# jackhwalters/DCS-Net

Measured on AMD Instinct MI355X. Metric: STFT frames/sec (train fwd+bwd+Adam), higher is better.
Workload: dtype f32

## Files before the change

### dcs-net_amd/csrc/lstm.hip

```cpp
#include "dcs_common.h"

namespace {

typedef float v2f __attribute__((ext_vector_type(2)));

__device__ __forceinline__ float fast_tanh(float x) {
    return 1.f - 2.f * __builtin_amdgcn_rcpf(__builtin_amdgcn_exp2f(x * 2.885390081777927f) + 1.f);
}

__device__ __forceinline__ void step_barrier() { asm volatile("s_waitcnt lgkmcnt(0)\n\ts_barrier" ::: "memory"); }

template <int CTRL>
__device__ __forceinline__ float quad_dpp(float v) { return dcs_dpp_term<CTRL, 0xf>(v); }
__device__ __forceinline__ float quad_bcast0(float v) { return quad_dpp<0x00>(v); }
__device__ __forceinline__ float quad_bcast1(float v) { return quad_dpp<0x55>(v); }
__device__ __forceinline__ float quad_bcast2(float v) { return quad_dpp<0xAA>(v); }
__device__ __forceinline__ float quad_bcast3(float v) { return quad_dpp<0xFF>(v); }
__device__ __forceinline__ float quad_sum(float v) {
    v += quad_dpp<0xB1>(v);
    v += quad_dpp<0x4E>(v);
    return v;
}

template <int H, bool SAVE>
// ... 152 lines not shown
}

extern "C" int dcs_lstm_layer_fwd_bias(const float* gx, const float* w_hh, const float* bias_a, const float* bias_b, float* out,
                                       float* gates_save, float* c_save, float* hprev_save, int n_sets, int seqs_per_set, int S,
                                       int Hdim, long stride_set, long stride_n, long stride_t, dcs_stream_t stream) {
    if (!gx || !w_hh || !out || n_sets <= 0 || seqs_per_set <= 0 || S <= 0 || (Hdim != 64 && Hdim != 128)) return DCS_ERR_BADARG;
    if ((gates_save == nullptr) != (c_save == nullptr)) return DCS_ERR_BADARG;
    if (bias_b && !bias_a) return DCS_ERR_BADARG;
    const int NS = n_sets * seqs_per_set;
    dim3 grid(NS * 2);
    if (Hdim == 128 && gates_save)
        DCS_LAUNCH((lstm_rec_fwd_kernel<128, true>), grid, dim3(512), 0, dcs_stream(stream), gx, w_hh, out, gates_save,
                           c_save, hprev_save, S, seqs_per_set, stride_set, stride_n, stride_t, bias_a, bias_b);
    else if (Hdim == 128)
        DCS_LAUNCH((lstm_rec_fwd_kernel<128, false>), grid, dim3(512), 0, dcs_stream(stream), gx, w_hh, out, gates_save,
                           c_save, hprev_save, S, seqs_per_set, stride_set, stride_n, stride_t, bias_a, bias_b);
    else if (gates_save)
        DCS_LAUNCH((lstm_rec_fwd_kernel<64, true>), grid, dim3(256), 0, dcs_stream(stream), gx, w_hh, out, gates_save,
                           c_save, hprev_save, S, seqs_per_set, stride_set, stride_n, stride_t, bias_a, bias_b);
    else
        DCS_LAUNCH((lstm_rec_fwd_kernel<64, false>), grid, dim3(256), 0, dcs_stream(stream), gx, w_hh, out, gates_save,
                           c_save, hprev_save, S, seqs_per_set, stride_set, stride_n, stride_t, bias_a, bias_b);
    DCS_CHECK_LAUNCH();
    return DCS_OK;
}

extern "C" int dcs_lstm_layer_fwd(const float* gx, const float* w_hh, float* out, float* gates_save, float* c_save,
                                  float* hprev_save, int n_sets, int seqs_per_set, int S, int Hdim, long stride_set, long stride_n,
                                  long stride_t, dcs_stream_t stream) {
    return dcs_lstm_layer_fwd_bias(gx, w_hh, nullptr, nullptr, out, gates_save, c_save, hprev_save, n_sets, seqs_per_set, S, Hdim,
                                   stride_set, stride_n, stride_t, stream);
}


namespace {
__global__ __launch_bounds__(256) void lstm_combine_fwd_kernel(const float* __restrict__ o, float2* __restrict__ out, long n) {
    const long i = (long)blockIdx.x * 256 + threadIdx.x;
    if (i >= n) return;
    const float rr = o[i], ir = o[n + i], ri = o[2 * n + i], ii = o[3 * n + i];
    out[i] = make_float2(rr - ii, ir + ri);
}
__global__ __launch_bounds__(256) void lstm_combine_bwd_kernel(const float2* __restrict__ g, float* __restrict__ g_o, long n) {
    DCS_PRIO_CRITICAL();
    const long i = (long)blockIdx.x * 256 + threadIdx.x;
    if (i >= n) return;
    const float2 v = g[i];
    g_o[i] = v.x; g_o[n + i] = v.y; g_o[2 * n + i] = v.y; g_o[3 * n + i] = -v.x;
}
__global__ __launch_bounds__(256) void lstm_param_grads_kernel(const float* __restrict__ part, const float* __restrict__ b_part,
                                                                float* __restrict__ g_whh, float* __restrict__ g_bih,
                                                                float* __restrict__ g_bhh, int CK, int seqs, int H, int w_blocks,
                                                                const float* __restrict__ part_ih, float* __restrict__ g_wih,
                                                                int CK_ih, long MN_ih, int ih_blocks, int ih_first) {
    if ((int)blockIdx.x >= ih_first) {
        const int bx = blockIdx.x - ih_first, s_ = bx / ih_blocks;
        const long i = (long)(bx % ih_blocks) * 256 + threadIdx.x;
        if (i >= MN_ih) return;
        const float* q = part_ih + (long)s_ * CK_ih * MN_ih + i;
        float a = 0.f;
#pragma unroll 8
        for (int c = 0; c < CK_ih; ++c) a += q[(long)c * MN_ih];
        g_wih[s_ * MN_ih + i] += a;
        return;
    }
    const int WH = 4 * H * H, nW = 4 * WH;
    if ((int)blockIdx.x < w_blocks) {
// ... 168 lines not shown
```

### dcs-net_amd/dcsnet/_lib.py

```python
import ctypes
import os

_HERE = os.path.dirname(os.path.abspath(__file__))
LIB_PATH = os.environ.get('DCS_LIB_PATH') or os.path.join(os.path.dirname(_HERE), 'lib', 'libdcsnet_hip.so')

ACT_NONE, ACT_RELU, ACT_LRELU, ACT_SIGMOID = 0, 1, 2, 3

_P = ctypes.c_void_p
_I = ctypes.c_int
_L = ctypes.c_long
_F = ctypes.c_float
_U64 = ctypes.c_ulonglong



class AttentionItem(ctypes.Structure):
    _fields_ = [(n, _P) for n in ('x', 'w1', 'w2', 'wsa', 'sa_bias', 'ca', 'pooled', 'hidden', 'sp', 'sa', 'y', 'g_out',
                                  'wsa_bwd', 'g_pre', 'g_sp', 'g_x', 'g_fc0_r', 'g_fc0_i', 'g_fc2_r', 'g_fc2_i')] + \
               [(n, _I) for n in ('H', 'W', 'C', 'Ch')] + [('g_pooled', _P)]


class SnapshotItem(ctypes.Structure):
    _fields_ = [('src', _P), ('words', _L), ('dst_word', _L), ('is_f32', _I), ('pad_', _I)]

# ... 22 lines not shown
    'dcs_cconv2d_bwd_weight_workspace_bytes': (_L, [_I] * 14),
    'dcs_cconv2d_bwd_weight': (_I, [_P] * 8 + [_L] + [_I] * 15 + [_P]),
    'dcs_cbn_workspace_bytes': (_L, [_L, _I]),
    'dcs_cbn_fwd': (_I, [_P] * 9 + [_L, _L, _I, _F, _F, _I, _I, _F, _U64, _P, _P]),
    'dcs_cbn_fwd_slabs': (_I, [_P] * 9 + [_I, _I, _P, _L, _I, _F, _F, _I, _F, _U64, _P, _P]),
    'dcs_ca_pool_chunks': (_I, [_L, _I]),
    'dcs_cbn_fwd_slabs_pool': (_I, [_P] * 9 + [_I, _I, _P, _P, _L, _I, _L, _I, _F, _F, _I, _P]),
    'dcs_channel_attention_fc_fwd': (_I, [_P] * 6 + [_I, _L, _I, _I, _P]),
    'dcs_cbn_bwd_workspace_bytes': (_L, [_L, _I]),
    'dcs_cbn_bwd': (_I, [_P] * 9 + [_L, _L, _I, _I, _I, _F, _U64, _P, _P]),
    'dcs_cbn_bwd_add': (_I, [_P] * 9 + [_L, _L, _I, _I, _I, _F, _U64, _P, _P, _F, _L, _P, _P]),
    'dcs_ca_workspace_bytes': (_L, [_I, _L, _I]),
    'dcs_channel_attention_fwd': (_I, [_P] * 7 + [_L, _I, _L, _I, _I, _P]),
    'dcs_spatial_pool_fwd': (_I, [_P, _P, _P, _I, _L, _I, _P]),
    'dcs_attention_apply_fwd': (_I, [_P, _P, _P, _P, _I, _L, _I, _F, _U64, _P, _P]),
    'dcs_rattention_workspace_bytes': (_L, [_I, _L, _I]),
    'dcs_rattention_fwd': (_I, [_P] * 8 + [_L] + [_I] * 6 + [_P]),
    'dcs_rattention_train_workspace_bytes': (_L, [_I, _L, _I, _I]),
    'dcs_rattention_pool_fwd': (_I, [_P] * 8 + [_L] + [_I] * 5 + [_P]),
    'dcs_rattention_apply_fwd': (_I, [_P] * 4 + [_I] * 4 + [_P]),
    'dcs_rattention_apply_bwd': (_I, [_P] * 8 + [_L] + [_I] * 4 + [_P]),
    'dcs_rattention_pool_bwd': (_I, [_P] * 11 + [_I] + [_P, _L] + [_I] * 5 + [_P]),
    'dcs_attention_bwd_sa': (_I, [_P] * 5 + [_I, _L, _I, _F, _U64, _P, _P]),
    'dcs_attention_bwd_workspace_bytes': (_L, [_I, _L, _I, _I]),
    'dcs_attention_bwd_x': (_I, [_P] * 16 + [_L, _I, _L, _I, _I, _F, _U64, _P, _P]),
    'dcs_attention_bwd_fc_weights': (_I, [_P, _L, _P, _P, _P, _P, _P, _P, _I, _L, _I, _I, _P]),
    'dcs_attention_fwd_batched_workspace_bytes': (_L, [_I, _P, _I]),
    'dcs_attention_fwd_batched': (_I, [_I, _P, _P, _L, _I, _P]),
    'dcs_attention_bwd_batched_workspace_bytes': (_L, [_I, _P, _I]),
    'dcs_attention_bwd_batched': (_I, [_I, _P, _P, _L, _I, _P]),
    'dcs_lstm_layer_fwd': (_I, [_P] * 6 + [_I, _I, _I, _I, _L, _L, _L, _P]),
    'dcs_lstm_layer_fwd_bias': (_I, [_P, _P, _P, _P, _P, _P, _P, _P, _I, _I, _I, _I, _L, _L, _L, _P]),
    'dcs_lstm_layer_bwd': (_I, [_P] * 6 + [_I] * 4 + [_P]),
    'dcs_dropout_fwd': (_I, [_P, _P, _L, _F, _U64, _P, _P]),
    'dcs_complex_act_fwd': (_I, [_P, _P, _L, _I, _P]),
    'dcs_complex_upsample_fwd': (_I, [_P, _P, _I, _I, _I, _I, _I, _I, _P]),
    'dcs_tapsum_fwd': (_I, [_P, _P, _P, _P] + [_I] * 10 + [_P]),
    'dcs_cconv_up2_single_fwd': (_I, [_P] * 6 + [_I] * 6 + [_P]),
    'dcs_cconv_up2_single_bwd_data': (_I, [_P] * 4 + [_I] * 6 + [_P]),
    'dcs_cconv_up2_single_bwd_weight_workspace_bytes': (_L, []),
    'dcs_cconv_up2_single_bwd_weight': (_I, [_P] * 7 + [_I, _P, _L] + [_I] * 5 + [_P]),
    'dcs_tapsum_bwd_workspace_bytes': (_L, []),
    'dcs_tapsum_bwd': (_I, [_P, _P, _P, _P, _P, _L] + [_I] * 10 + [_P]),
    'dcs_bound_crm_fwd': (_I, [_P, _P, _L, _F, _P]),
    'dcs_bound_mask_apply_fwd': (_I, [_P, _P, _P, _P, _P, _L, _F, _P]),
    'dcs_bound_mask_apply_bwd': (_I, [_P] * 6 + [_L, _F, _P]),
    'dcs_bound2_mask_apply_fwd': (_I, [_P] * 6 + [_L, _F, _F, _U64, _P, _P]),
    'dcs_bound2_mask_apply_bwd': (_I, [_P] * 7 + [_L, _F, _F, _U64, _P, _P]),
    'dcs_bound2_apply_polar_frames_fwd': (_I, [_P] * 4 + [_I] * 4 + [_F, _F, _U64, _P, _P]),
    'dcs_bound2_apply_polar_frames_bwd': (_I, [_P] * 5 + [_I] * 4 + [_F, _I, _F, _U64, _P, _P]),
    'dcs_complex_abs_f32': (_I, [_P, _P, _L, _P]),
    'dcs_rmask_apply_polar_frames_fwd': (_I, [_P] * 4 + [_I] * 4 + [_F, _I, _P]),
    'dcs_rmask_apply_polar_frames_bwd': (_I, [_P] * 5 + [_I] * 4 + [_F, _I, _I, _P]),
    'dcs_irfft512_frames': (_I, [_P, _P, _L, _P]),
    'dcs_rfft512_frames': (_I, [_P, _P, _L, _P]),
    'dcs_rfft512_ola_frames': (_I, [_P, _P, _P, _P, _I, _I, _I, _F, _P]),
    'dcs_irfft512_ola_frames': (_I, [_P, _P, _P, _P, _I, _I, _I, _F, _P]),
    'dcs_polar_frames_fwd': (_I, [_P, _P, _I, _I, _I, _I, _F, _P]),
    'dcs_polar_frames_bwd': (_I, [_P, _P, _P, _I, _I, _I, _I, _F, _I, _P]),
    'dcs_istft_envelope': (_I, [_P, _P, _I, _I, _I, _P]),
    'dcs_istft_ola_fwd': (_I, [_P, _P, _P, _P, _I, _I, _I, _I, _F, _P]),
    'dcs_istft_ola_bwd': (_I, [_P, _P, _P, _P, _I, _I, _I, _I, _F, _P]),
    'dcs_stft_frames_fwd': (_I, [_P, _P, _P, _P, _I, _I, _I, _I, _I, _P]),
    'dcs_stft_bins_fwd': (_I, [_P, _P, _I, _I, _I, _F, _P]),
    'dcs_sisnr_fwd': (_I, [_P, _P, _P, _P, _I, _I, _F, _P]),
    'dcs_sisnr_bwd': (_I, [_P, _P, _P, _P, _F, _P, _I, _I, _P]),
# ... 100 lines not shown
```

### dcs-net_amd/dcsnet/functional.py

```python
import os
import weakref

import torch

from . import _derived
from . import ops
from .ops import ACT_NONE, ACT_RELU, ACT_LRELU, ACT_SIGMOID, to_nhwc, from_nhwc
from ._lib import DcsHipError

_PACKED = _derived.Derived(capacity=512)


def bump_param_generation():
    _derived.bump_generation()
    ops.pack_plan_invalidate()


def note_state_update():
    _derived.bump_generation()


state_generation = _derived.generation


# ... 478 lines not shown


def _project_bwd(g_gx, w_ih, shared):
    G8, K = w_ih.shape[1], w_ih.shape[2]
    M = g_gx.shape[1]
    if not (ops.gemm_ok(M, K, G8, 2, True) and g_gx.is_contiguous() and w_ih.is_contiguous()):
        if shared:
            g_inp = torch.mm(g_gx[0], w_ih[0])
            return g_inp.addmm_(g_gx[1], w_ih[1])
        return torch.bmm(g_gx, w_ih)
    if shared:
        g_inp = torch.empty((M, K), dtype=torch.float32, device=g_gx.device)
        return ops.gemm_f32(g_gx, w_ih, g_inp, M, K, G8, G8, K, K, False, nseg=2, a_seg=M * G8, b_seg=G8 * K)
    g_inp = torch.empty((2, M, K), dtype=torch.float32, device=g_gx.device)
    return ops.gemm_f32(g_gx, w_ih, g_inp, M, K, G8, G8, K, K, False, nbatch=2, a_batch=M * G8, b_batch=G8 * K, c_batch=M * K)


class _ProjectFn(torch.autograd.Function):

    @staticmethod
    def forward(ctx, inp, w_ih):
        ctx.save_for_backward(inp, w_ih)
        return _project(inp, w_ih, shared=inp.dim() == 2, per_set=True)

    @staticmethod
    def backward(ctx, g):
        inp, w_ih = ctx.saved_tensors
        g = g.contiguous()
        g_inp = _project_bwd(g, w_ih, shared=inp.dim() == 2) if ctx.needs_input_grad[0] else None
        g_w = torch.matmul(g.transpose(1, 2), inp) if ctx.needs_input_grad[1] else None
        return g_inp, g_w


class _LstmLayerFn(torch.autograd.Function):

    @staticmethod
    def forward(ctx, inp, anchor, st, B2, S):
        w_ih, w_hh = st['weight_ih'][0], st['weight_hh'][0]
        need = inp.requires_grad or anchor.requires_grad
        ctx.planes = 0
        if inp.is_complex():
            zr = torch.view_as_real(inp)
            G8, K = w_ih.shape[1], w_ih.shape[2]
            ctx.planes = R0 = zr.shape[0] * zr.shape[1]
            gx = torch.empty((2 * R0, 2 * G8), dtype=torch.float32, device=inp.device)
            ops.gemm_f32(zr, w_ih, gx, 2 * R0, 2 * G8, K, K, K, 2 * G8, True, a_planes=R0)
            inp = zr
            G4 = G8 // 2
            strides = (G8, S * 2 * G8, 2 * G8)
        elif inp.dim() == 2:
            G8 = w_ih.shape[1]
            gx = _project(inp, w_ih, shared=True)
            G4 = G8 // 2
            strides = (G8, S * 2 * G8, 2 * G8)
        else:
            gx = _project(inp, w_ih, shared=False)
            G4 = gx.shape[-1] // 2
            strides = (B2 * S * 2 * G4, S * 2 * G4, 2 * G4)
        out, gates, c, hprev = ops.lstm_layer(gx, w_hh, 2, B2, S, strides, need, True,
                                              bias=(st['bias_ih'][0], st['bias_hh'][0]))
        ctx.st, ctx.dims = st, (B2, S)
        if need:
            ctx.save_for_backward(inp, hprev, gates, c)
        return out

    @staticmethod
    def backward(ctx, g_out):
        global sink_hits
        inp, hprev, gates, c = ctx.saved_tensors
        st, (B2, S) = ctx.st, ctx.dims
        w_ih, w_hh = st['weight_ih'][0], st['weight_hh'][0]
        H = w_hh.shape[-1]
        NT = B2 * S
# ... 67 lines not shown
    return st


_LSTM_OPERANDS = _derived.Derived()


def _lstm_layer_operands(sets, layer):
    names = [f'_l{layer}', f'_l{layer}_reverse']
    params = [getattr(m, k + n) for m in sets for n in names for k in ('weight_ih', 'weight_hh', 'bias_ih', 'bias_hh')]

    def make():
        w_ih = torch.stack([torch.cat([getattr(m, 'weight_ih' + n) for n in names]) for m in sets])
        bias = torch.stack([torch.cat([getattr(m, 'bias_ih' + n) + getattr(m, 'bias_hh' + n) for n in names])
                            for m in sets])
        w_hh = torch.stack([torch.stack([getattr(m, 'weight_hh' + n) for n in names]) for m in sets]).contiguous()
        return w_ih, bias, w_hh
    cacheable = not (torch.is_grad_enabled() and any(p.requires_grad for p in params))
    if not cacheable:
        return make()
    return _LSTM_OPERANDS.get(sets[0], layer, params, lambda: tuple(t.detach() for t in make()))


def complex_lstm(z, real_lstm, imag_lstm):
    if not (real_lstm.bidirectional and real_lstm.batch_first and real_lstm.hidden_size == 64):
        raise DcsHipError('complex_lstm: the HIP path implements the reference geometry '
                          '(bidirectional, batch_first, hidden 64: c_network.py:118-123)')
    B, S, I = z.shape
    sets = (real_lstm, imag_lstm)
    inp = None
    stacked = _stacked_lstm(real_lstm) if torch.is_grad_enabled() else None
    in_place = (stacked is not None and z.is_contiguous() and (B * S) % 64 == 0 and I % 64 == 0
                and ops.gemm_ok(2 * B * S, 16 * real_lstm.hidden_size, I, 1, True) and ops.gemm_ok(2 * B * S, I, 8 * real_lstm.hidden_size, 2, True)
                and stacked[0]['weight_ih'][0].is_contiguous() and stacked[0]['weight_ih'][1].is_contiguous())
    x2 = None if in_place else torch.view_as_real(z).permute(3, 0, 1, 2).reshape(2 * B * S, I)
    for layer in range(real_lstm.num_layers):
        if stacked is not None:
            out = _LstmLayerFn.apply((z if in_place else x2) if layer == 0 else inp, real_lstm.weight_ih_l0, stacked[layer], 2 * B, S)
            inp = out.view(2, 2 * B * S, -1)
            continue
        w_ih, bias, w_hh = _lstm_layer_operands(sets, layer)
        if not (torch.is_grad_enabled() and ((x2 if layer == 0 else inp).requires_grad or bias.requires_grad or w_ih.requires_grad)):
            if layer == 0:
                G8 = w_ih.shape[1]
                gx = _project(x2, w_ih.contiguous(), shared=True, train=False)
                strides = (G8, S * 2 * G8, 2 * G8)
            else:
                gx = _project(inp, w_ih.contiguous(), shared=False, train=False)
                strides = (2 * B * S * gx.shape[-1], S * gx.shape[-1], gx.shape[-1])
            out = ops.lstm_layer(gx, w_hh.contiguous(), 2, 2 * B, S, strides, False, bias=(bias.contiguous(), None))[0]
            inp = out.view(2, 2 * B * S, -1)
            continue
        gx = _ProjectFn.apply(x2 if layer == 0 else inp, w_ih) + bias.unsqueeze(1)
        out = _LstmRecFn.apply(gx.view(2, 2 * B, S, 2, -1), w_hh)
        inp = out.view(2, 2 * B * S, -1)
    o = inp.view(2, 2 * B, S, -1)
    if torch.is_grad_enabled() and o.requires_grad:
        return _LstmCombineFn.apply(o, B)
    return ops.lstm_combine(o.contiguous(), B)


class _TapSumFn(torch.autograd.Function):

    @staticmethod
    def forward(ctx, z, ksize, up, pad, b_r, b_i):
        ctx.cfg = (tuple(z.shape), tuple(ksize), tuple(up), tuple(pad))
        ctx.bias = b_r is not None
        ctx.sinks = (_sink(b_r), _sink(b_i)) if ctx.bias else (None, None)
        return ops.tapsum(z, ksize, up, pad, bias=(b_r, b_i) if ctx.bias else None)

    @staticmethod
    def backward(ctx, g):
        shape, ksize, up, pad = ctx.cfg
        g = g.contiguous()
        if not ctx.bias:
            return ops.tapsum(shape, ksize, up, pad, backward=True, grad=g), None, None, None, None, None
        new = lambda: torch.empty(1, dtype=torch.float32, device=g.device)
        dst = tuple(s_ if s_ is not None else new() for s_ in ctx.sinks)
        gz = ops.tapsum(shape, ksize, up, pad, backward=True, grad=g, bias_grad=dst)
        gb = tuple(None if s_ is not None else d for d, s_ in zip(dst, ctx.sinks))
        return gz, None, None, None, gb[0], gb[1]


class _TapRowsConvFn(torch.autograd.Function):

    @staticmethod
# ... 442 lines not shown
```

### dcs-net_amd/dcsnet/ops.py

```python
import os as _os
import torch

from . import _lib
from ._lib import ACT_NONE, ACT_RELU, ACT_LRELU, ACT_SIGMOID, check, ptr, cur_stream


def _chk(t, name, dims=None, act=False):
    if t is None:
        return
    if not t.is_cuda:
        raise _lib.DcsHipError(f'{name}: expected a CUDA (HIP) tensor; the HIP path has no CPU fallback')
    if t.dtype != torch.float32 and not (act and t.dtype == torch.bfloat16):
        raise _lib.DcsHipError(f'{name}: expected float32{" or bfloat16" if act else ""}, got {t.dtype}')
    if not t.is_contiguous():
        raise _lib.DcsHipError(f'{name}: expected a contiguous tensor')
    if dims is not None and t.dim() != dims:
        raise _lib.DcsHipError(f'{name}: expected {dims} dims, got shape {tuple(t.shape)}')


def _sym(name, *acts):
    dts = {t.dtype for t in acts if t is not None}
    if len(dts) > 1:
        raise _lib.DcsHipError(f'{name}: activation tensors of different dtypes {sorted(str(d) for d in dts)}')
    bf = dts == {torch.bfloat16}
# ... 615 lines not shown
        g_pre = torch.empty((B, H, W, 1, 2), dtype=torch.float32, device=dev)
        g_sp = torch.empty((B, H, W, 2, 2), dtype=torch.float32, device=dev)
        g_x = torch.empty_like(x)
        g_pooled = torch.empty((B, C, 2), dtype=torch.float32, device=dev) if split else None
        blocks.append(dict(x=x, w1=sv['w1'], w2=sv['w2'], ca=sv['ca'], pooled=sv['pooled'], hidden=sv['hidden'], sa=sv['sa'],
                           g_out=g, wsa_bwd=wb, g_pre=g_pre, g_sp=g_sp, g_x=g_x, g_fc0_r=fo[0], g_fc0_i=fo[1], g_fc2_r=fo[2],
                           g_fc2_i=fo[3], H=H, W=W, C=C, Ch=sv['hidden'].shape[1], **({'g_pooled': g_pooled} if split else {})))
        res.append((g_x, g_pre, g_pooled))
    items = _attention_items(blocks)
    n = len(blocks)
    nbytes = lib.dcs_attention_bwd_batched_workspace_bytes(n, items, B)
    if nbytes < 0:
        raise _lib.DcsHipError('attention_blocks_bwd: unsupported block geometry')
    ws = _workspace(nbytes, dev)
    check(_sym('dcs_attention_bwd_batched', *g_outs, *[sv['x'] for sv in saved])(n, items, ptr(ws), ws.numel(), B, cur_stream()), 'dcs_attention_bwd_batched')
    return res


def lstm_layer(gx, w_hh, n_sets, seqs_per_set, S, strides, save=False, save_hprev=False, bias=None):
    _chk(gx, 'gx')
    _chk(w_hh, 'w_hh', 4)
    H = w_hh.shape[-1]
    NS = n_sets * seqs_per_set
    out = torch.empty((NS, S, 2 * H), dtype=torch.float32, device=gx.device)
    gates = torch.empty((NS, S, 2, 4 * H), dtype=torch.float32, device=gx.device) if save else None
    c = torch.empty((NS, S, 2, H), dtype=torch.float32, device=gx.device) if save else None
    hprev = torch.empty((NS, S, 2, H), dtype=torch.float32, device=gx.device) if save and save_hprev else None
    ba, bb = (None, None) if bias is None else bias
    _chk(ba, 'bias_a')
    _chk(bb, 'bias_b')
    check(_lib.load().dcs_lstm_layer_fwd_bias(ptr(gx), ptr(w_hh), ptr(ba), ptr(bb), ptr(out), ptr(gates), ptr(c), ptr(hprev),
                                              n_sets, seqs_per_set, S, H, strides[0], strides[1], strides[2], cur_stream()),
          'dcs_lstm_layer_fwd_bias')
    return (out, gates, c, hprev) if save_hprev else (out, gates, c)


def lstm_layer_bwd(g_out, gates, c, w_hh, n_sets, seqs_per_set, S, bias_part=False):
    _chk(g_out, 'g_out', 3)
    _chk(gates, 'gates', 4)
    _chk(c, 'c', 4)
    _chk(w_hh, 'w_hh', 4)
    g_pre = torch.empty_like(gates)
    part = torch.empty((gates.shape[0], 2, gates.shape[-1]), dtype=torch.float32, device=gates.device) if bias_part else None
    check(_lib.load().dcs_lstm_layer_bwd(ptr(g_out), ptr(gates), ptr(c), ptr(w_hh), ptr(g_pre), ptr(part), n_sets,
                                         seqs_per_set, S, w_hh.shape[-1], cur_stream()), 'dcs_lstm_layer_bwd')
    return (g_pre, part) if bias_part else g_pre


def dropout(x, drop_p, seed, out=None):
    _chk(x, 'x')
    y = torch.empty_like(x) if out is None else out
    check(_lib.load().dcs_dropout_fwd(ptr(x), ptr(y), x.numel(), float(drop_p), int(seed), ptr(SEED_STATE), cur_stream()),
          'dcs_dropout_fwd')
    return y


def complex_act(x, act, out=None):
    _chk(x, 'x')
    y = torch.empty_like(x) if out is None else out
    check(_lib.load().dcs_complex_act_fwd(ptr(x), ptr(y), x.numel(), act, cur_stream()), 'dcs_complex_act_fwd')
    return y


def complex_upsample(x, up):
    _chk(x, 'x', 5)
    B, H, W, C, _ = x.shape
# ... 888 lines not shown
```

### include/dcsnet_hip.h

```cpp
#ifndef DCSNET_HIP_H
#define DCSNET_HIP_H

#ifdef __cplusplus
extern "C" {
#endif

typedef void* dcs_stream_t;

#define DCS_OK              0
#define DCS_ERR_BADARG     (-1)
#define DCS_ERR_LAUNCH     (-2)
#define DCS_ERR_WORKSPACE  (-3)

#define DCS_ACT_NONE   0
#define DCS_ACT_RELU   1
#define DCS_ACT_LRELU  2
#define DCS_ACT_SIGMOID 3

int         dcs_abi_version(void);
const char* dcs_error_string(int code);

long dcs_packed_weight_floats(int Cout, int Cin, int kh, int kw, int up_f, int up_t);
int dcs_pack_conv_weight(const float* w_r, const float* w_i, const float* b_r, const float* b_i,
                         float* wp, float* bias_out,
// ... 132 lines not shown
                             float* pooled, void* workspace, long workspace_bytes, int B, int H, int W, int C, int Ch,
                             dcs_stream_t stream);
int  dcs_rattention_apply_fwd(const float* x, const float* ca, const float* sa, float* y, int B, int H, int W, int C,
                              dcs_stream_t stream);
int  dcs_rattention_apply_bwd(const float* gy, const float* x, const float* ca, const float* sa, float* gx, float* g_sa,
                              float* g_ca, void* workspace, long workspace_bytes, int B, int H, int W, int C,
                              dcs_stream_t stream);
int  dcs_rattention_pool_bwd(const float* g_pooled, const float* g_ca, const float* x, const float* ca, const float* mx,
                             const float* hid, const float* w1, const float* w2, float* gx, float* gw1, float* gw2,
                             int accumulate, void* workspace, long workspace_bytes, int B, int H, int W, int C, int Ch,
                             dcs_stream_t stream);

int  dcs_attention_bwd_sa(const float* x, const float* g_out, const float* ca, const float* sa, float* g_pre,
                          int B, long HW, int C, float drop_p, unsigned long long seed, const unsigned long long* seed_dev, dcs_stream_t stream);
long dcs_attention_bwd_workspace_bytes(int B, long HW, int C, int Ch);
int  dcs_attention_bwd_x(const float* x, const float* g_out, const float* ca, const float* sa, const float* g_sp,
                         const float* pooled, const float* hidden, const float* w1, const float* w2,
                         float* g_x, float* g_fc0_r, float* g_fc0_i, float* g_fc2_r, float* g_fc2_i, float* g_pooled,
                         void* workspace, long workspace_bytes, int B, long HW, int C, int Ch,
                         float drop_p, unsigned long long seed, const unsigned long long* seed_dev, dcs_stream_t stream);
int dcs_attention_bwd_fc_weights(const void* workspace, long workspace_bytes, const float* pooled, const float* hidden,
                                 float* g_fc0_r, float* g_fc0_i, float* g_fc2_r, float* g_fc2_i, int B, long HW, int C, int Ch,
                                 dcs_stream_t stream);

int dcs_lstm_layer_fwd(const float* gx, const float* w_hh, float* out, float* gates_save, float* c_save,
                       float* hprev_save, int n_sets, int seqs_per_set, int S, int H, long stride_set, long stride_n, long stride_t,
                       dcs_stream_t stream);

int dcs_lstm_layer_fwd_bias(const float* gx, const float* w_hh, const float* bias_a, const float* bias_b, float* out,
                            float* gates_save, float* c_save, float* hprev_save, int n_sets, int seqs_per_set, int S,
                            int Hdim, long stride_set, long stride_n, long stride_t, dcs_stream_t stream);
int dcs_lstm_layer_bwd(const float* g_out, const float* gates, const float* c_save, const float* w_hh,
                       float* g_pre, float* g_bias_part, int n_sets, int seqs_per_set, int S, int H, dcs_stream_t stream);

int dcs_lstm_whh_grad(const float* g_pre, const float* h_prev, float* part, int NT, int CK, int H, dcs_stream_t stream);
int dcs_atb_chunks(const float* A, const float* B, float* part, long a_lo, long a_hi, long b_lo, long b_hi, int nlo, int nhi,
                   int lda, int ldb, int M, int N, int R, int CK, dcs_stream_t stream);
int dcs_chunk_sum_acc(const float* part, float* out, long o_lo, long o_hi, int nlo, int nhi, int CK, long MN,
                      dcs_stream_t stream);
int dcs_atb_chunks_strided(const float* A, const float* B, float* part, long a_lo, long a_hi, long b_lo, long b_hi, int nlo,
                           int nhi, int lda, int ldb, int b_es, int M, int N, int R, int CK, dcs_stream_t stream);
int dcs_gemm_f32(const float* A, const float* B, float* C, int M, int N, int K, int lda, int ldb, int ldc, int b_transposed,
                 int nseg, long a_seg, long b_seg, int nbatch, long a_batch, long b_batch, long c_batch, int a_planes,
                 int c_planes, dcs_stream_t stream);
int dcs_lstm_combine_fwd(const float* o, float* out, long n, dcs_stream_t stream);
int dcs_lstm_combine_bwd(const float* g, float* g_o, long n, dcs_stream_t stream);
int dcs_lstm_param_grads(const float* part, const float* b_part, float* g_whh, float* g_bih, float* g_bhh, int CK,
                         int seqs_per_set, int H, dcs_stream_t stream);
int dcs_lstm_param_grads_ih(const float* part, const float* b_part, float* g_whh, float* g_bih, float* g_bhh, int CK,
                            int seqs_per_set, int H, const float* part_ih, float* g_wih, int CK_ih, long MN_ih, int nsets,
                            dcs_stream_t stream);

int dcs_dropout_fwd(const float* x, float* y, long n, float drop_p, unsigned long long seed,
                    const unsigned long long* seed_dev, dcs_stream_t stream);

int dcs_complex_act_fwd(const float* x, float* y, long n_floats, int act, dcs_stream_t stream);
int dcs_complex_upsample_fwd(const float* x, float* y, int B, int H, int W, int C, int up_f, int up_t,
                             dcs_stream_t stream);

int dcs_tapsum_fwd(const float* z, float* y, const float* b_r, const float* b_i, int B, int Hs, int Ws, int CT,
                   int kh, int kw, int up_f, int up_t, int pad_f, int pad_t, dcs_stream_t stream);
long dcs_tapsum_bwd_workspace_bytes(void);
int dcs_tapsum_bwd(const float* gy, float* gz, float* gb_r, float* gb_i, void* workspace, long workspace_bytes,
                   int B, int Hs, int Ws, int CT, int kh, int kw, int up_f, int up_t, int pad_f, int pad_t,
                   dcs_stream_t stream);

// ... 228 lines not shown
```

Baseline: 2.492 million.

## Fuse LSTM input projection into recurrent kernel with MFMA chunk pipelining

```diff
diff --git a/dcs-net_amd/csrc/lstm.hip b/dcs-net_amd/csrc/lstm.hip
--- a/dcs-net_amd/csrc/lstm.hip
+++ b/dcs-net_amd/csrc/lstm.hip
@@ -208,6 +208,224 @@
                                    stride_set, stride_n, stride_t, stream);
 }
 
+namespace {
+typedef float f32x4p __attribute__((ext_vector_type(4)));
+constexpr int LP_TC = 16, LP_K = 128, LP_PITCH = 4 * 64 + 4;
+enum { FORM_BOUNDARY = 0, FORM_WAVES = 1, FORM_STEPS = 2 };
+
+struct LstmProjP {
+    const float* inp; const float* wih; const float* whh; const float* bias_a; const float* bias_b;
+    float* out; float* gates_save; float* c_save; float* hprev_save;
+    long in_set;
+    int S, seqs_per_set;
+};
+
+template <int FORM, bool SAVE, bool AP>
+__global__ __launch_bounds__(FORM == FORM_WAVES ? 512 : 256) void lstm_proj_fwd_kernel(LstmProjP p) {
+    constexpr int H = 64, G4 = 4 * H, Q = H / 4, TC = LP_TC, K = LP_K, NB = K / 16;
+    static_assert(4 * NB == 2 * TC, "two (tile, k-block) units per piece");
+    __shared__ __attribute__((aligned(16))) float pre_s[2][TC * LP_PITCH];
+    __shared__ __attribute__((aligned(16))) float h_s[2][H];
+    const int S = p.S;
+    const int wave = __builtin_amdgcn_readfirstlane(threadIdx.x >> 6), lane = threadIdx.x & 63, pw = wave & 3;
+    const bool rec = FORM != FORM_WAVES || wave < 4;
+    const int t = threadIdx.x & 255, u = t >> 2, gate = t & 3, j = gate * H + u;
+    const int n = blockIdx.x >> 1, dir = blockIdx.x & 1;
+    const int set = n / p.seqs_per_set, ns = n % p.seqs_per_set;
+    const int t0 = dir ? S - 1 : 0, dt = dir ? -1 : 1;
+    const int nchunks = (S + TC - 1) / TC;
+
+    float w[4][Q];
+    float c = 0.f, hprev = 0.f;
+    float bias_a = 0.f, bias_b = 0.f;
+    if (rec && p.bias_a) bias_a = p.bias_a[(set * 2 + dir) * G4 + j];
+    if (rec && p.bias_b) bias_b = p.bias_b[(set * 2 + dir) * G4 + j];
+    auto rec_setup = [&]() {
+#pragma unroll
+        for (int g = 0; g < 4; ++g) {
+            const float4* wr = reinterpret_cast<const float4*>(p.whh + ((long)(set * 2 + dir) * G4 + g * H + u) * H + gate * Q);
+#pragma unroll
+            for (int k = 0; k < Q / 4; ++k) {
+                const float4 v = wr[k];
+                w[g][4 * k] = v.x; w[g][4 * k + 1] = v.y; w[g][4 * k + 2] = v.z; w[g][4 * k + 3] = v.w;
+            }
+        }
+        if (t < H) h_s[0][t] = 0.f;
+    };
+    const bool is_g = gate == 2;
+    auto step = [&](int s, const float* prow) {
+        const int tt = t0 + s * dt, cur = s & 1;
+        const float pre = *prow + (bias_a + bias_b);
+        v2f acc[4] = {v2f{0.f, 0.f}, v2f{0.f, 0.f}, v2f{0.f, 0.f}, v2f{0.f, 0.f}};
+        const float4* h4 = reinterpret_cast<const float4*>(h_s[cur] + gate * Q);
+#pragma unroll
+        for (int k = 0; k < Q / 4; ++k) {
+            const float4 hv = h4[k];
+#pragma unroll
+            for (int g = 0; g < 4; ++g) {
+                acc[g] = __builtin_elementwise_fma(v2f{w[g][4 * k], w[g][4 * k + 1]}, v2f{hv.x, hv.y}, acc[g]);
+                acc[g] = __builtin_elementwise_fma(v2f{w[g][4 * k + 2], w[g][4 * k + 3]}, v2f{hv.z, hv.w}, acc[g]);
+            }
+        }
+        const float s0 = quad_sum(acc[0].x + acc[0].y), s1 = quad_sum(acc[1].x + acc[1].y);
+        const float s2 = quad_sum(acc[2].x + acc[2].y), s3 = quad_sum(acc[3].x + acc[3].y);
+        const float a = pre + (gate == 0 ? s0 : (gate == 1 ? s1 : (gate == 2 ? s2 : s3)));
+        const float th = fast_tanh(is_g ? a : 0.5f * a);
+        const float act = is_g ? th : fmaf(0.5f, th, 0.5f);
+        if (SAVE) p.gates_save[(((long)n * S + tt) * 2 + dir) * G4 + j] = act;
+        const float ig = quad_bcast0(act), fg = quad_bcast1(act), gg = quad_bcast2(act), og = quad_bcast3(act);
+        c = fmaf(fg, c, ig * gg);
+        const float h = og * fast_tanh(c);
+        if (gate == 0) h_s[cur ^ 1][u] = h;
+        p.out[((long)n * S + tt) * (2 * H) + dir * H + u] = h;
+        if (SAVE) {
+            p.c_save[(((long)n * S + tt) * 2 + dir) * H + u] = c;
+            if (p.hprev_save) p.hprev_save[(((long)n * S + tt) * 2 + dir) * H + u] = hprev;
+        }
+        hprev = h;
+    };
+
+    float bw[4][NB][4], av[NB][4];
+    f32x4p pacc[4];
+    const int li = lane & 15, kk = lane >> 4;
+    auto load_a = [&](int cidx, int blk) {
+        const int s_ = cidx * TC + li, s = s_ < S ? s_ : S - 1, tt = t0 + s * dt;
+        if (AP) {
+            const int Bh = p.seqs_per_set >> 1, part = ns / Bh;
+            const float* q = p.inp + (((long)(ns % Bh) * S + tt) * K + 4 * kk) * 2 + blk * 32;
+            const float4 x = *reinterpret_cast<const float4*>(q), y = *reinterpret_cast<const float4*>(q + 4);
+            av[blk][0] = part ? x.y : x.x; av[blk][1] = part ? x.w : x.z; av[blk][2] = part ? y.y : y.x; av[blk][3] = part ? y.w : y.z;
+        } else {
+            const float4 v = *reinterpret_cast<const float4*>(p.inp + set * p.in_set + ((long)ns * S + tt) * K + 4 * kk + blk * 16);
+            av[blk][0] = v.x; av[blk][1] = v.y; av[blk][2] = v.z; av[blk][3] = v.w;
+        }
+    };
+    auto piece = [&](int i, int buf, int refill) {
+        const f32x4p z = {0.f, 0.f, 0.f, 0.f};
+#pragma unroll
+        for (int m = 0; m < 8; ++m) {
+            const int un = 2 * i + (m & 1), jj = m >> 1, blk = un >> 2, q = un & 3;
+            pacc[q] = __builtin_amdgcn_mfma_f32_16x16x4f32(av[blk][jj], bw[q][blk][jj], blk == 0 && jj == 0 ? z : pacc[q], 0, 0, 0);
+        }
+#pragma unroll
+        for (int un = 2 * i; un < 2 * i + 2; ++un) {
+            const int blk = un >> 2, q = un & 3;
+            if (q == 3) load_a(refill, blk);
+            if (blk == NB - 1) {
+                float* o = pre_s[buf] + (4 * kk) * LP_PITCH + 64 * pw + 16 * q + li;
+#pragma unroll
+                for (int r = 0; r < 4; ++r) o[r * LP_PITCH] = pacc[q][r];
+            }
+        }
+    };
+    auto prod_load = [&]() {
+#pragma unroll
+        for (int blk = 0; blk < NB; ++blk) load_a(0, blk);
+#pragma unroll
+        for (int blk = 0; blk < NB; ++blk)
+#pragma unroll
+            for (int q = 0; q < 4; ++q) {
+                const int tc = 64 * pw + 16 * q + li, jr = (tc & 3) * H + (tc >> 2);
+                const float4 v = *reinterpret_cast<const float4*>(p.wih + ((long)(set * 2 + dir) * G4 + jr) * K + 4 * kk + blk * 16);
+                bw[q][blk][0] = v.x; bw[q][blk][1] = v.y; bw[q][blk][2] = v.z; bw[q][blk][3] = v.w;
+            }
+    };
+    auto prod_chunk0 = [&]() {
+#pragma unroll
+        for (int i = 0; i < TC; ++i) piece(i, 0, 1);
+    };
+    auto steps = [&](int cidx) {
+        const int s0 = cidx * TC, nc = S - s0 < TC ? S - s0 : TC;
+        const float* prow = pre_s[cidx & 1] + t;
+        for (int i = 0; i < nc; ++i) {
+            step(s0 + i, prow + i * LP_PITCH);
+            step_barrier();
+        }
+    };
+
+    if (FORM == FORM_WAVES) {
+        if (rec) {
+            DCS_PRIO_CRITICAL();
+            rec_setup();
+            __syncthreads();
+            for (int cidx = 0; cidx < nchunks; ++cidx) steps(cidx);
+        } else {
+            prod_load();
+            prod_chunk0();
+            __syncthreads();
+            for (int cidx = 0; cidx < nchunks; ++cidx) {
+                if (cidx + 1 < nchunks) {
+#pragma unroll
+                    for (int i = 0; i < TC; ++i) {
+                        piece(i, (cidx & 1) ^ 1, cidx + 2);
+                        step_barrier();
+                    }
+                } else {
+                    const int nc = S - cidx * TC;
+                    for (int i = 0; i < nc; ++i) step_barrier();
+                }
+            }
+        }
+        return;
+    }
+    prod_load();
+    rec_setup();
+    prod_chunk0();
+    __syncthreads();
+    for (int cidx = 0; cidx < nchunks; ++cidx) {
+        const bool next = cidx + 1 < nchunks;
+        if (FORM == FORM_STEPS && next) {
+            const float* prow = pre_s[cidx & 1] + t;
+#pragma unroll
+            for (int i = 0; i < TC; ++i) {
+                piece(i, (cidx & 1) ^ 1, cidx + 2);
+                step(cidx * TC + i, prow + i * LP_PITCH);
+                step_barrier();
+            }
+            continue;
+        }
+        steps(cidx);
+        if (next) {
+#pragma unroll
+            for (int i = 0; i < TC; ++i) piece(i, (cidx & 1) ^ 1, cidx + 2);
+            step_barrier();
+        }
+    }
+}
+
+template <int FORM>
+void lstm_proj_launch(const LstmProjP& p, bool save, bool planes, int nwg, hipStream_t st) {
+    const dim3 grid(nwg), block(FORM == FORM_WAVES ? 512 : 256);
+    if (save && planes) DCS_LAUNCH((lstm_proj_fwd_kernel<FORM, true, true>), grid, block, 0, st, p);
+    else if (save) DCS_LAUNCH((lstm_proj_fwd_kernel<FORM, true, false>), grid, block, 0, st, p);
+    else if (planes) DCS_LAUNCH((lstm_proj_fwd_kernel<FORM, false, true>), grid, block, 0, st, p);
+    else DCS_LAUNCH((lstm_proj_fwd_kernel<FORM, false, false>), grid, block, 0, st, p);
+}
+}
+
+extern "C" int dcs_lstm_layer_fwd_proj(const float* inp, const float* w_ih, const float* w_hh, const float* bias_a,
+                                       const float* bias_b, float* out, float* gates_save, float* c_save, float* hprev_save,
+                                       int n_sets, int seqs_per_set, int S, int Hdim, int in_dim, long in_set_stride, int planes,
+                                       int form, dcs_stream_t stream) {
+    if (!inp || !w_ih || !w_hh || !out || n_sets <= 0 || seqs_per_set <= 0 || S <= 0) return DCS_ERR_BADARG;
+    if (Hdim != 64 || in_dim != LP_K) return DCS_ERR_BADARG;
+    if ((gates_save == nullptr) != (c_save == nullptr) || (hprev_save && !gates_save)) return DCS_ERR_BADARG;
+    if (bias_b && !bias_a) return DCS_ERR_BADARG;
+    if (planes && ((seqs_per_set & 1) || in_set_stride != 0)) return DCS_ERR_BADARG;
+    if (in_set_stride < 0 || (in_set_stride & 3) || ((uintptr_t)inp & 15) || ((uintptr_t)w_ih & 15) || ((uintptr_t)w_hh & 15))
+        return DCS_ERR_BADARG;
+    if (form < 0 || form > 3 || (long)n_sets * seqs_per_set * 2 > 0x7fffffffL) return DCS_ERR_BADARG;
+    LstmProjP p{inp, w_ih, w_hh, bias_a, bias_b, out, gates_save, c_save, hprev_save, in_set_stride, S, seqs_per_set};
+    const int nwg = n_sets * seqs_per_set * 2;
+    const hipStream_t st = dcs_stream(stream);
+    const int f = form == 0 ? 3 : form;
+    if (f == 1) lstm_proj_launch<FORM_BOUNDARY>(p, gates_save != nullptr, planes != 0, nwg, st);
+    else if (f == 2) lstm_proj_launch<FORM_WAVES>(p, gates_save != nullptr, planes != 0, nwg, st);
+    else lstm_proj_launch<FORM_STEPS>(p, gates_save != nullptr, planes != 0, nwg, st);
+    DCS_CHECK_LAUNCH();
+    return DCS_OK;
+}
+
 
 namespace {
 __global__ __launch_bounds__(256) void lstm_combine_fwd_kernel(const float* __restrict__ o, float2* __restrict__ out, long n) {
diff --git a/dcs-net_amd/dcsnet/_lib.py b/dcs-net_amd/dcsnet/_lib.py
--- a/dcs-net_amd/dcsnet/_lib.py
+++ b/dcs-net_amd/dcsnet/_lib.py
@@ -78,6 +78,7 @@
     'dcs_lstm_layer_fwd': (_I, [_P] * 6 + [_I, _I, _I, _I, _L, _L, _L, _P]),
     'dcs_lstm_layer_fwd_bias': (_I, [_P, _P, _P, _P, _P, _P, _P, _P, _I, _I, _I, _I, _L, _L, _L, _P]),
     'dcs_lstm_layer_bwd': (_I, [_P] * 6 + [_I] * 4 + [_P]),
+    'dcs_lstm_layer_fwd_proj': (_I, [_P] * 9 + [_I] * 5 + [_L, _I, _I, _P]),
     'dcs_dropout_fwd': (_I, [_P, _P, _L, _F, _U64, _P, _P]),
     'dcs_complex_act_fwd': (_I, [_P, _P, _L, _I, _P]),
     'dcs_complex_upsample_fwd': (_I, [_P, _P, _I, _I, _I, _I, _I, _I, _P]),
diff --git a/dcs-net_amd/dcsnet/functional.py b/dcs-net_amd/dcsnet/functional.py
--- a/dcs-net_amd/dcsnet/functional.py
+++ b/dcs-net_amd/dcsnet/functional.py
@@ -534,6 +534,37 @@
         return g_inp, g_w
 
 
+class _LstmLayerProjFn(torch.autograd.Function):
+
+    @staticmethod
+    def forward(ctx, inp, w_ih, bias, w_hh, B2, S):
+        need = any(t.requires_grad for t in (inp, w_ih, bias, w_hh))
+        out, gates, c = ops.lstm_layer_proj(inp, w_ih, w_hh, 2, B2, S, need, False, bias=(bias, None))
+        ctx.dims = (B2, S)
+        if need:
+            ctx.save_for_backward(inp, w_ih, w_hh, out, gates, c)
+        return out
+
+    @staticmethod
+    def backward(ctx, g_out):
+        inp, w_ih, w_hh, out, gates, c = ctx.saved_tensors
+        B2, S = ctx.dims
+        H = w_hh.shape[-1]
+        g_pre = ops.lstm_layer_bwd(g_out.contiguous(), gates, c, w_hh, 2, B2, S)
+        g_gx = g_pre.view(2, B2 * S, 8 * H)
+        g_inp = _project_bwd(g_gx, w_ih, shared=inp.dim() == 2) if ctx.needs_input_grad[0] else None
+        g_wih = torch.matmul(g_gx.transpose(1, 2), inp) if ctx.needs_input_grad[1] else None
+        g_bias = g_gx.sum(1) if ctx.needs_input_grad[2] else None
+        g_whh = None
+        if ctx.needs_input_grad[3]:
+            g_pre5, o = g_pre.view(2, B2, S, 2, 4 * H), out.view(2, B2, S, 2, H)
+            h_prev = torch.zeros_like(o)
+            h_prev[:, :, 1:, 0] = o[:, :, :-1, 0]
+            h_prev[:, :, :-1, 1] = o[:, :, 1:, 1]
+            g_whh = torch.einsum('sntdj,sntdk->sdjk', g_pre5, h_prev)
+        return g_inp, g_wih, g_bias, g_whh, None, None
+
+
 class _LstmLayerFn(torch.autograd.Function):
 
     @staticmethod
@@ -541,6 +572,16 @@
         w_ih, w_hh = st['weight_ih'][0], st['weight_hh'][0]
         need = inp.requires_grad or anchor.requires_grad
         ctx.planes = 0
+        bias = (st['bias_ih'][0], st['bias_hh'][0])
+        lat = torch.view_as_real(inp) if inp.is_complex() else inp
+        if ops.lstm_fused_ok(w_hh.shape[-1], w_ih.shape[2], 4 * B2, S, lat, w_ih, w_hh, *bias):
+            if inp.is_complex():
+                ctx.planes = lat.shape[0] * lat.shape[1]
+            out, gates, c, hprev = ops.lstm_layer_proj(lat, w_ih, w_hh, 2, B2, S, need, True, bias=bias, planes=inp.is_complex())
+            ctx.st, ctx.dims = st, (B2, S)
+            if need:
+                ctx.save_for_backward(lat, hprev, gates, c)
+            return out
         if inp.is_complex():
             zr = torch.view_as_real(inp)
             G8, K = w_ih.shape[1], w_ih.shape[2]
@@ -674,17 +715,28 @@
     in_place = (stacked is not None and z.is_contiguous() and (B * S) % 64 == 0 and I % 64 == 0
                 and ops.gemm_ok(2 * B * S, 16 * real_lstm.hidden_size, I, 1, True) and ops.gemm_ok(2 * B * S, I, 8 * real_lstm.hidden_size, 2, True)
                 and stacked[0]['weight_ih'][0].is_contiguous() and stacked[0]['weight_ih'][1].is_contiguous())
-    x2 = None if in_place else torch.view_as_real(z).permute(3, 0, 1, 2).reshape(2 * B * S, I)
+    x2_ = []
+
+    def x2():
+        if not x2_:
+            x2_.append(torch.view_as_real(z).permute(3, 0, 1, 2).reshape(2 * B * S, I))
+        return x2_[0]
     for layer in range(real_lstm.num_layers):
         if stacked is not None:
-            out = _LstmLayerFn.apply((z if in_place else x2) if layer == 0 else inp, real_lstm.weight_ih_l0, stacked[layer], 2 * B, S)
+            out = _LstmLayerFn.apply((z if in_place else x2()) if layer == 0 else inp, real_lstm.weight_ih_l0, stacked[layer], 2 * B, S)
             inp = out.view(2, 2 * B * S, -1)
             continue
         w_ih, bias, w_hh = _lstm_layer_operands(sets, layer)
-        if not (torch.is_grad_enabled() and ((x2 if layer == 0 else inp).requires_grad or bias.requires_grad or w_ih.requires_grad)):
+        if not (torch.is_grad_enabled() and ((z if layer == 0 else inp).requires_grad or bias.requires_grad or w_ih.requires_grad)):
+            w_ih, w_hh, bias = w_ih.contiguous(), w_hh.contiguous(), bias.contiguous()
+            lat = inp if layer else (torch.view_as_real(z) if z.is_contiguous() else x2())
+            if ops.lstm_fused_ok(real_lstm.hidden_size, w_ih.shape[2], 8 * B, S, lat, w_ih, w_hh, bias):
+                out = ops.lstm_layer_proj(lat, w_ih, w_hh, 2, 2 * B, S, False, bias=(bias, None), planes=lat.dim() == 4)[0]
+                inp = out.view(2, 2 * B * S, -1)
+                continue
             if layer == 0:
                 G8 = w_ih.shape[1]
-                gx = _project(x2, w_ih.contiguous(), shared=True, train=False)
+                gx = _project(x2(), w_ih.contiguous(), shared=True, train=False)
                 strides = (G8, S * 2 * G8, 2 * G8)
             else:
                 gx = _project(inp, w_ih.contiguous(), shared=False, train=False)
@@ -692,7 +744,12 @@
             out = ops.lstm_layer(gx, w_hh.contiguous(), 2, 2 * B, S, strides, False, bias=(bias.contiguous(), None))[0]
             inp = out.view(2, 2 * B * S, -1)
             continue
-        gx = _ProjectFn.apply(x2 if layer == 0 else inp, w_ih) + bias.unsqueeze(1)
+        lat = x2() if layer == 0 else inp
+        if ops.lstm_fused_ok(real_lstm.hidden_size, w_ih.shape[2], 8 * B, S, lat, w_ih, w_hh, bias):
+            out = _LstmLayerProjFn.apply(lat, w_ih, bias, w_hh, 2 * B, S)
+            inp = out.view(2, 2 * B * S, -1)
+            continue
+        gx = _ProjectFn.apply(lat, w_ih) + bias.unsqueeze(1)
         out = _LstmRecFn.apply(gx.view(2, 2 * B, S, 2, -1), w_hh)
         inp = out.view(2, 2 * B * S, -1)
     o = inp.view(2, 2 * B, S, -1)
diff --git a/dcs-net_amd/dcsnet/ops.py b/dcs-net_amd/dcsnet/ops.py
--- a/dcs-net_amd/dcsnet/ops.py
+++ b/dcs-net_amd/dcsnet/ops.py
@@ -671,6 +671,48 @@
     check(_lib.load().dcs_lstm_layer_fwd_bias(ptr(gx), ptr(w_hh), ptr(ba), ptr(bb), ptr(out), ptr(gates), ptr(c), ptr(hprev),
                                               n_sets, seqs_per_set, S, H, strides[0], strides[1], strides[2], cur_stream()),
           'dcs_lstm_layer_fwd_bias')
+    return (out, gates, c, hprev) if save_hprev else (out, gates, c)
+
+
+LSTM_FUSED_PROJ = _os.environ.get('DCS_LSTM_FUSED_PROJ', '1') != '0'
+
+
+def lstm_fused_ok(H, n_in, n_wg, S, *operands):
+    return (LSTM_FUSED_PROJ and H == 64 and n_in == 128 and n_wg >= 128 and n_wg * S >= 4096
+            and all(t.is_contiguous() and t.dtype == torch.float32 and t.data_ptr() % 16 == 0 for t in operands))
+
+
+def lstm_layer_proj(inp, w_ih, w_hh, n_sets, seqs_per_set, S, save=False, save_hprev=False, bias=None, planes=False, form=0):
+    _chk(inp, 'inp')
+    _chk(w_ih, 'w_ih', 3)
+    _chk(w_hh, 'w_hh', 4)
+    H, n_in = w_hh.shape[-1], w_ih.shape[-1]
+    if tuple(w_ih.shape) != (n_sets, 8 * H, n_in) or tuple(w_hh.shape) != (n_sets, 2, 4 * H, H):
+        raise _lib.DcsHipError(f'lstm_layer_proj: w_ih {tuple(w_ih.shape)} / w_hh {tuple(w_hh.shape)} for {n_sets} sets')
+    if planes:
+        want, in_set = (seqs_per_set // 2, S, n_in, 2), 0
+        ok = seqs_per_set % 2 == 0 and tuple(inp.shape) == want
+    elif inp.dim() == 2:
+        want, in_set = (seqs_per_set * S, n_in), 0
+        ok = tuple(inp.shape) == want
+    else:
+        want, in_set = (n_sets, seqs_per_set * S, n_in), seqs_per_set * S * n_in
+        ok = tuple(inp.shape) == want
+    if not ok:
+        raise _lib.DcsHipError(f'lstm_layer_proj: inp {tuple(inp.shape)}, expected {want}')
+    NS = n_sets * seqs_per_set
+    out = torch.empty((NS, S, 2 * H), dtype=torch.float32, device=inp.device)
+    gates = torch.empty((NS, S, 2, 4 * H), dtype=torch.float32, device=inp.device) if save else None
+    c = torch.empty((NS, S, 2, H), dtype=torch.float32, device=inp.device) if save else None
+    hprev = torch.empty((NS, S, 2, H), dtype=torch.float32, device=inp.device) if save and save_hprev else None
+    ba, bb = (None, None) if bias is None else bias
+    for nm, b in (('bias_a', ba), ('bias_b', bb)):
+        _chk(b, nm)
+        if b is not None and b.numel() != n_sets * 8 * H:
+            raise _lib.DcsHipError(f'lstm_layer_proj: {nm} {tuple(b.shape)}, expected [{n_sets}, {8 * H}]')
+    check(_lib.load().dcs_lstm_layer_fwd_proj(ptr(inp), ptr(w_ih), ptr(w_hh), ptr(ba), ptr(bb), ptr(out), ptr(gates), ptr(c),
+                                              ptr(hprev), n_sets, seqs_per_set, S, H, n_in, in_set, 1 if planes else 0, form,
+                                              cur_stream()), 'dcs_lstm_layer_fwd_proj')
     return (out, gates, c, hprev) if save_hprev else (out, gates, c)
 
 
diff --git a/include/dcsnet_hip.h b/include/dcsnet_hip.h
--- a/include/dcsnet_hip.h
+++ b/include/dcsnet_hip.h
@@ -188,6 +188,9 @@
                             int Hdim, long stride_set, long stride_n, long stride_t, dcs_stream_t stream);
 int dcs_lstm_layer_bwd(const float* g_out, const float* gates, const float* c_save, const float* w_hh,
                        float* g_pre, float* g_bias_part, int n_sets, int seqs_per_set, int S, int H, dcs_stream_t stream);
+int dcs_lstm_layer_fwd_proj(const float* inp, const float* w_ih, const float* w_hh, const float* bias_a, const float* bias_b,
+                            float* out, float* gates_save, float* c_save, float* hprev_save, int n_sets, int seqs_per_set,
+                            int S, int H, int in, long in_set_stride, int planes, int form, dcs_stream_t stream);
 
 int dcs_lstm_whh_grad(const float* g_pre, const float* h_prev, float* part, int NT, int CK, int H, dcs_stream_t stream);
 int dcs_atb_chunks(const float* A, const float* B, float* part, long a_lo, long a_hi, long b_lo, long b_hi, int nlo, int nhi,
```

Result: no change. 2.513 million (median of 6 runs) (+0.8%).
